# frgfm/Holocron

Measured on NVIDIA H100. Metric: images/sec RepVGG-A0 224^2 bf16 train, higher is better.
Workload: dtype bf16

## Files before the change

holocron_b200/csrc/conv_common.cuh:

```cuda
#pragma once
#include <cuda_runtime.h>
#include <type_traits>
#include "common.cuh"
#include "tc_common.cuh"
#include "tmap.cuh"

namespace conv {

constexpr int kThreads = 384;
constexpr int kConsumers = 256;

__device__ __forceinline__ void consumer_sync() { asm volatile("bar.sync 1, 256;" ::: "memory"); }

struct Ring {
  int stage = 0;
  uint32_t phase = 0;
  __device__ __forceinline__ void next(int n) {
    if (++stage == n) { stage = 0; phase ^= 1; }
  }
  __device__ __forceinline__ static Ring at(int k, int n) { return Ring{k % n, (uint32_t)(k / n) & 1}; }
};

__device__ __forceinline__ void add_residual16(uint4& val, const uint4& rv, bool relu) {
  __nv_bfloat162* a = reinterpret_cast<__nv_bfloat162*>(&val);
  const __nv_bfloat162* b = reinterpret_cast<const __nv_bfloat162*>(&rv);
#pragma unroll
  for (int jj = 0; jj < 4; ++jj) {
    float2 fa = __bfloat1622float2(a[jj]), fb = __bfloat1622float2(b[jj]);
    fa.x += fb.x; fa.y += fb.y;
    if (relu) { fa.x = hb::relu_nan(fa.x); fa.y = hb::relu_nan(fa.y); }
    a[jj] = __floats2bfloat162_rn(fa.x, fa.y);
  }
}

__device__ __forceinline__ void accum_pair(float4& s, const uint8_t* staged) {
  const float2 f = __bfloat1622float2(*reinterpret_cast<const __nv_bfloat162*>(staged));
  s.x += f.x; s.y += f.y; s.z = fmaf(f.x, f.x, s.z); s.w = fmaf(f.y, f.y, s.w);
}
__device__ __forceinline__ float2 fold_stats(const float4* scratch, int rgs, int npairs, int c) {
  const int pr = c >> 1, hi = c & 1;
  float sv = 0.f, qv = 0.f;
  for (int rg = 0; rg < rgs; ++rg) {
    const float4 v = scratch[rg * npairs + pr];
    sv += hi ? v.y : v.x;
    qv += hi ? v.w : v.z;
  }
  return make_float2(sv, qv);
}
__device__ __forceinline__ void store_stats(float* stats, int slot, int Cout, int channel, float2 v) {
  *reinterpret_cast<float2*>(stats + ((size_t)slot * Cout + channel) * 2) = v;
}

template <auto kKernel, typename... Args>
cudaError_t launch(int grid, size_t smem_bytes, cudaStream_t stream, const Args&... args) {
  static const cudaError_t attr =
      cudaFuncSetAttribute(kKernel, cudaFuncAttributeMaxDynamicSharedMemorySize, 227 * 1024);
  if (attr != cudaSuccess) return attr;
  kKernel<<<grid, kThreads, smem_bytes, stream>>>(args...);
  g_hb_launches.fetch_add(1, std::memory_order_relaxed);
  return cudaGetLastError();
}

template <int kStep, int kMax, int W = kStep, typename F>
cudaError_t dispatch_width(int w, F&& f) {
  if (w == W) return f(std::integral_constant<int, W>{});
  if constexpr (W + kStep <= kMax) return dispatch_width<kStep, kMax, W + kStep>(w, f);
  else return cudaErrorInvalidValue;
}

}

int hb_conv_rows_try(const void* x, const void* w, void* y, const float* bias, const void* residual, int N, int H, int W,
                     int Cin, int Cout, int act, int num_ctas, cudaStream_t stream, int nextra, const void* const* xe,
                     const void* const* we, float* stats, int* stat_slots);
int hb_wgrad_rows_try(const void* x, const void* dy, const void* dy1, float* ws, size_t ws_bytes, int N, int H, int W,
                      int Cin, int Cout, int num_ctas, cudaStream_t stream, int* slices_out);
size_t hb_wgrad_rows_workspace_bytes(int N, int H, int W, int Cin, int Cout, int R, int S, int stride, int pad, int dil,
                                     int num_ctas, int has_b1);
```

holocron_b200/csrc/conv_fprop.cu:

```cuda
#include <stdlib.h>
#include "conv_common.cuh"
#include "holocron_b200.h"

namespace {

using namespace tc;
using namespace conv;

constexpr int kBM = 128;
constexpr int kBK = 64;
constexpr int kMmaK = 16;
constexpr int kProducerRegs = 40;
constexpr int kConsumerRegs = 232;
constexpr int kABytes = kBM * kBK * 2;
constexpr int kSmemMax = 227 * 1024;

struct FpropParams {
  int m_total;
  int Ho, Wo;
  int stride, pad_h, pad_w, dil;
  int R, S;
  int Cin, Cout;
  int num_m_tiles, num_n_tiles;
  int cblocks;
  int ksteps_last;
  int e_mode, e_cblocks, e_ksteps_last;
  int nout;
  int stages;
  int b_stage_bytes;
  int out_pitch;
  int a_mode;
  int act;
  __nv_bfloat16* y;
  __nv_bfloat16* y2;
  float* stats;
  float* stats2;
  const float* bias;
  const __nv_bfloat16* residual;
  const float* norm_mean;
  const float* norm_rstd;
  const float* norm_wsum;
  int scatter, OH, OW, o_step, o_a, o_b;
};

template <bool kStats, int BN>
__global__ void __launch_bounds__(kThreads, 1)
conv_fprop_kernel(const __grid_constant__ CUtensorMap tmA, const __grid_constant__ CUtensorMap tmB,
                  const __grid_constant__ CUtensorMap tmA2, const __grid_constant__ CUtensorMap tmB2, const FpropParams p) {
  extern __shared__ __align__(1024) uint8_t smem_raw[];
  uint8_t* smem = reinterpret_cast<uint8_t*>((reinterpret_cast<uintptr_t>(smem_raw) + 1023) & ~uintptr_t(1023));
  const int stage_bytes = kABytes + p.b_stage_bytes;
  uint8_t* sout = smem + (size_t)p.stages * stage_bytes;
  const size_t sout_bytes = (((size_t)kBM * p.out_pitch + 15) & ~(size_t)15) + kBM * sizeof(long long);
  uint64_t* full_bar = reinterpret_cast<uint64_t*>(sout + sout_bytes);
  uint64_t* empty_bar = full_bar + p.stages;

  const int warp = threadIdx.x >> 5;
  const int lane = threadIdx.x & 31;

  if (warp == 0 && lane == 0) {
    prefetch_tmap(&tmA);
    prefetch_tmap(&tmB);
    if (p.e_mode) { prefetch_tmap(&tmB2); if (p.e_mode == 1) prefetch_tmap(&tmA2); }
    for (int i = 0; i < p.stages; ++i) { mbar_init(&full_bar[i], 1); mbar_init(&empty_bar[i], kConsumers / 32); }
    fence_barrier_init();
  }
  __syncthreads();

  const int n_tile = blockIdx.x % p.num_n_tiles;
  const int m_first = blockIdx.x / p.num_n_tiles, m_step = gridDim.x / p.num_n_tiles;
  const int kblocks = p.R * p.S * p.cblocks;
  const uint32_t tx_bytes = kABytes + BN * 128;

  if (warp < 4) {
    regs_release<kProducerRegs>();
    if (warp == 0 && lane == 0) {
      Ring ring;
      for (int m_tile = m_first; m_tile < p.num_m_tiles; m_tile += m_step) {
        const int m0 = m_tile * kBM;
        const int q0 = m0 % p.Wo, p0 = (m0 / p.Wo) % p.Ho, n0 = m0 / (p.Wo * p.Ho);
        const int base_w = q0 * p.stride - p.pad_w, base_h = p0 * p.stride - p.pad_h;
        for (int tap = 0; tap < p.R * p.S; ++tap) {
          const int r = tap / p.S, s = tap % p.S;
          for (int cb = 0; cb < p.cblocks; ++cb) {
            uint64_t* bar = &full_bar[ring.stage];
            mbar_wait(&empty_bar[ring.stage], ring.phase ^ 1);
            uint8_t* sa = smem + (size_t)ring.stage * stage_bytes;
            uint8_t* sb = sa + kABytes;
            mbar_arrive_expect_tx(bar, tx_bytes);
            if (p.a_mode == 1)
              tma_load_im2col_4d(&tmA, bar, sa, cb * kBK, base_w, base_h, n0, (uint16_t)(s * p.dil), (uint16_t)(r * p.dil));
            else
              tma_load_2d(&tmA, bar, sa, cb * kBK, m0);
            tma_load_3d(&tmB, bar, sb, cb * kBK, tap, n_tile * BN);
            ring.next(p.stages);
          }
        }
        for (int cb = 0; cb < p.e_cblocks; ++cb) {
          uint64_t* bar = &full_bar[ring.stage];
          mbar_wait(&empty_bar[ring.stage], ring.phase ^ 1);
          uint8_t* sa = smem + (size_t)ring.stage * stage_bytes;
          uint8_t* sb = sa + kABytes;
          mbar_arrive_expect_tx(bar, tx_bytes);
          if (p.e_mode == 1)
            tma_load_2d(&tmA2, bar, sa, cb * kBK, m0);
          else if (p.a_mode == 1)
            tma_load_im2col_4d(&tmA, bar, sa, cb * kBK, base_w, base_h, n0, (uint16_t)((p.S / 2) * p.dil),
                               (uint16_t)((p.R / 2) * p.dil));
          else
            tma_load_2d(&tmA, bar, sa, cb * kBK, m0);
          tma_load_3d(&tmB2, bar, sb, cb * kBK, 0, n_tile * BN);
          ring.next(p.stages);
        }
      }
    }
    return;
  }

  regs_acquire<kConsumerRegs>();
  const int et = threadIdx.x - 128;
  const int wg = et >> 7;
  const int wet = et & 127;
  const int frow = 64 * wg + frag_row(wet);
  const int fcol = frag_col(wet);
  const uint32_t dhi = desc_hi(1024);
  const uint32_t a_lo0 = desc_lo(smem_u32(smem), 16) + (uint32_t)wg * ((64 * 128) >> 4);
  const uint32_t stage_lo = (uint32_t)stage_bytes >> 4;
  long long* row_off = reinterpret_cast<long long*>(sout + (((size_t)kBM * p.out_pitch + 15) & ~(size_t)15));
  const int gpo = (BN + 63) >> 6;
  const int ngroups = p.nout * gpo;
  float4 st[4];
#pragma unroll
  for (int gi = 0; gi < 4; ++gi) st[gi] = make_float4(0.f, 0.f, 0.f, 0.f);
  const int col_base = n_tile * BN;
  const int ncols_valid = min(BN, p.Cout - col_base);
  constexpr int kCols = BN <= 64 ? 2 * BN : BN;
  float acc[kCols / 2];
  Ring ring;

  for (int m_tile = m_first; m_tile < p.num_m_tiles; m_tile += m_step) {
    int prev = -1;
    auto next_block = [&](uint32_t& a_lo, uint32_t& b_lo) {
      mbar_wait(&full_bar[ring.stage], ring.phase);
      a_lo = a_lo0 + (uint32_t)ring.stage * stage_lo;
      b_lo = desc_lo(smem_u32(smem), 16) + (uint32_t)ring.stage * stage_lo + (kABytes >> 4);
    };
    auto retire_prev = [&]() {
      wgmma_wait<1>();
      if (prev >= 0 && lane == 0) mbar_arrive(&empty_bar[prev]);
      prev = ring.stage;
      ring.next(p.stages);
    };
    for (int kb = 0, cb = 0; kb < kblocks; ++kb) {
      uint32_t a_lo, b_lo;
      next_block(a_lo, b_lo);
      if (++cb == p.cblocks) {
        cb = 0;
        wgmma_group_ks<BN, 0, 0>(p.ksteps_last, acc, a_lo, b_lo, 2, dhi, kb != 0);
      } else {
        wgmma_group<BN, kBK / kMmaK, 0, 0>(acc, a_lo, b_lo, 2, dhi, kb != 0);
      }
      retire_prev();
    }
    for (int ecb = 0; ecb < p.e_cblocks; ++ecb) {
      uint32_t a_lo, b_lo;
      next_block(a_lo, b_lo);
      const int ks = (ecb == p.e_cblocks - 1) ? p.e_ksteps_last : kBK / kMmaK;
      if constexpr (BN <= 64) {
        if (p.e_mode == 2) wgmma_group_ks<BN, 0, 0>(ks, acc + BN / 2, a_lo, b_lo, 2, dhi, ecb != 0);
        else wgmma_group_ks<BN, 0, 0>(ks, acc, a_lo, b_lo, 2, dhi, 1u);
      } else {
        wgmma_group_ks<BN, 0, 0>(ks, acc, a_lo, b_lo, 2, dhi, 1u);
      }
      retire_prev();
    }
    wgmma_wait<0>();
    fence_regs(acc);
    if (lane == 0) mbar_arrive(&empty_bar[prev]);

    const int rows_valid = min(kBM, p.m_total - m_tile * kBM);
    float nm[2] = {0.f, 0.f}, nr[2] = {1.f, 1.f};
    if (p.norm_mean) {
#pragma unroll
      for (int h = 0; h < 2; ++h) {
        const int m_row = m_tile * kBM + frow + 8 * h;
        if (m_row < p.m_total) { nm[h] = __ldg(p.norm_mean + m_row); nr[h] = __ldg(p.norm_rstd + m_row); }
      }
    }
#pragma unroll 1
    for (int gi = 0; gi < ngroups; ++gi) {
      const int o = gi >= gpo ? 1 : 0;
      const int g0 = (gi - o * gpo) * 64;
      const int gw = min(64, BN - g0);
      __nv_bfloat16* yo = o ? p.y2 : p.y;
      const bool first = o == 0;
      const int cs0 = o * BN + g0;
      consumer_sync();
      if (gi == 0 && et < kBM) {
        const long long m = (long long)m_tile * kBM + et;
        if (!p.scatter) {
          row_off[et] = m * p.Cout;
        } else {
          const int j = (int)(m % p.Wo), i = (int)((m / p.Wo) % p.Ho), n = (int)(m / ((long long)p.Wo * p.Ho));
          row_off[et] = (((long long)n * p.OH + (long long)i * p.o_step + p.o_a) * p.OW + (long long)j * p.o_step + p.o_b) * p.Cout;
        }
      }
#pragma unroll
      for (int j = 0; j < kCols / 8; ++j) {
        const int cs = 8 * j + fcol;
        if (cs >= cs0 && cs < cs0 + gw) {
          const int cl = cs - cs0;
          const int col = col_base + g0 + cl;
          const bool ok = col < p.Cout;
#pragma unroll
          for (int h = 0; h < 2; ++h) {
            float f0 = acc[4 * j + 2 * h], f1 = acc[4 * j + 2 * h + 1];
            if (first && p.norm_mean && ok) {
              f0 = nr[h] * (f0 - nm[h] * __ldg(p.norm_wsum + col));
              f1 = nr[h] * (f1 - nm[h] * __ldg(p.norm_wsum + col + 1));
            }
            if (first && p.bias && ok) { f0 += __ldg(p.bias + col); f1 += __ldg(p.bias + col + 1); }
            if (first && p.act == 1 && !p.residual) { f0 = hb::relu_nan(f0); f1 = hb::relu_nan(f1); }
            *reinterpret_cast<__nv_bfloat162*>(sout + (size_t)(frow + 8 * h) * p.out_pitch + cl * 2) =
                __floats2bfloat162_rn(f0, f1);
          }
        }
      }
      consumer_sync();
      const int chunks_per_row = gw / 8;
      const int total_chunks = rows_valid * chunks_per_row;
      int r = et / chunks_per_row, c8 = et - r * chunks_per_row;
      const int dr = kConsumers / chunks_per_row, dc = kConsumers - dr * chunks_per_row;
      const __nv_bfloat16* resid = first ? p.residual : nullptr;
      if (!resid) {
        for (int ch = et; ch < total_chunks; ch += kConsumers) {
          if (g0 + c8 * 8 < ncols_valid) {
            const uint4 val = *reinterpret_cast<const uint4*>(sout + (size_t)r * p.out_pitch + c8 * 16);
            *reinterpret_cast<uint4*>(yo + (size_t)row_off[r] + col_base + g0 + c8 * 8) = val;
          }
          r += dr; c8 += dc;
          if (c8 >= chunks_per_row) { c8 -= chunks_per_row; ++r; }
        }
      } else {
        for (int ch = et; ch < total_chunks; ch += 4 * kConsumers) {
          size_t off[4];
          int sidx[4];
          uint4 rv[4];
          bool ok[4];
#pragma unroll
          for (int u = 0; u < 4; ++u) {
            ok[u] = (ch + u * kConsumers < total_chunks) && (g0 + c8 * 8 < ncols_valid);
            sidx[u] = r * p.out_pitch + c8 * 16;
            off[u] = ok[u] ? (size_t)row_off[r] + col_base + g0 + c8 * 8 : 0;
            if (ok[u]) rv[u] = *reinterpret_cast<const uint4*>(resid + off[u]);
            r += dr; c8 += dc;
            if (c8 >= chunks_per_row) { c8 -= chunks_per_row; ++r; }
          }
#pragma unroll
          for (int u = 0; u < 4; ++u) {
            if (!ok[u]) continue;
            uint4 val = *reinterpret_cast<const uint4*>(sout + sidx[u]);
            add_residual16(val, rv[u], p.act == 1);
            *reinterpret_cast<uint4*>(yo + off[u]) = val;
          }
        }
      }
      if (kStats && (o ? (p.stats2 != nullptr) : (p.stats != nullptr))) {
        const int npairs = gw >> 1, rgs = 128 / npairs;
        const int rg = wet / npairs, pr = wet - rg * npairs;
        const int row_end = min(64 * wg + 64, rows_valid);
        if (rg < rgs && g0 + pr * 2 < ncols_valid) {
          const uint8_t* sp = sout + pr * 4;
          float4 s = make_float4(0.f, 0.f, 0.f, 0.f);
          for (int rr = 64 * wg + rg; rr < row_end; rr += rgs) accum_pair(s, sp + (size_t)rr * p.out_pitch);
#pragma unroll
          for (int g = 0; g < 4; ++g)
            if (g == gi) { st[g].x += s.x; st[g].y += s.y; st[g].z += s.z; st[g].w += s.w; }
        }
      }
    }
  }
  if (kStats && (p.stats || p.stats2)) {
    const int slot = (blockIdx.x / p.num_n_tiles) * 2 + wg;
#pragma unroll
    for (int gi = 0; gi < 4; ++gi) {
      if (gi >= ngroups) break;
      const int o = gi >= gpo ? 1 : 0;
      float* so = o ? p.stats2 : p.stats;
      if (!so) continue;
      const int g0 = (gi - o * gpo) * 64;
      const int gw = min(64, BN - g0);
      const int npairs = gw >> 1, rgs = 128 / npairs;
      consumer_sync();
      float4* scratch = reinterpret_cast<float4*>(sout) + wg * 128;
      scratch[wet] = st[gi];
      consumer_sync();
      if (wet < gw && g0 + wet < ncols_valid)
        store_stats(so, slot, p.Cout, col_base + g0 + wet, fold_stats(scratch, rgs, npairs, wet));
    }
  }
}

struct FpropArgs {
  const void* x; const void* w; void* y; const float* bias; const void* residual;
  int N, H, W, Cin, Cout, R, S, stride;
  int pad_h, pad_w, pad_after_h, pad_after_w, dil, act, num_ctas;
  int Ho, Wo;
  int scatter, OH, OW, o_step, o_a, o_b;
  const void* xe; const void* we; int Ce;
  const void* w2; void* y2;
  float* stats; float* stats2; int* stat_slots;
  const float* norm_mean; const float* norm_rstd; const float* norm_wsum;
  cudaStream_t stream;
};

int fprop_launch(const FpropArgs& a) {
  const int Cin = a.Cin, Cout = a.Cout, R = a.R, S = a.S;
  const long long m_total_ll = (long long)a.N * a.Ho * a.Wo;
  if (a.Ho <= 0 || a.Wo <= 0 || m_total_ll <= 0 || m_total_ll > 0x7fffffffLL) return (int)cudaErrorInvalidValue;
  const bool dual = a.w2 != nullptr;
  const bool kext = a.xe != nullptr;
  if (dual && kext) return (int)cudaErrorInvalidValue;
  if (dual && (!a.y2 || a.scatter || !(R & 1) || !(S & 1))) return (int)cudaErrorInvalidValue;
  if (kext && (!a.we || a.Ce % 8 != 0 || a.scatter || !hb::aligned16(a.xe) || !hb::aligned16(a.we)))
    return (int)cudaErrorInvalidValue;
  FpropParams p{};
  p.m_total = (int)m_total_ll;
  p.Ho = a.Ho; p.Wo = a.Wo;
  p.stride = a.stride; p.pad_h = a.pad_h; p.pad_w = a.pad_w; p.dil = a.dil;
  p.R = R; p.S = S; p.Cin = Cin; p.Cout = Cout;
  p.scatter = a.scatter; p.OH = a.OH; p.OW = a.OW; p.o_step = a.o_step; p.o_a = a.o_a; p.o_b = a.o_b;
  p.num_m_tiles = (p.m_total + kBM - 1) / kBM;
  int grid = a.num_ctas > 0 ? a.num_ctas : HB_NUM_SMS;
  if (grid > HB_NUM_SMS * 4) grid = HB_NUM_SMS * 4;
  const int bn_max = dual ? 64 : 128;
  int BN = Cout;
  if (Cout > bn_max) {
    BN = bn_max;
    for (int c = bn_max; c >= 64; c -= 16) if (Cout % c == 0) { BN = c; break; }
    const int wide = dual || R * S == 1 || a.stats ? 0 : Cout <= 256 ? Cout : Cout % 256 == 0 ? 256 : Cout % 192 == 0 ? 192 : 0;
    if (wide && (long long)p.num_m_tiles * (Cout / wide) >= grid) BN = wide;
  }
  p.nout = dual ? 2 : 1;
  p.num_n_tiles = (Cout + BN - 1) / BN;
  p.cblocks = (Cin + kBK - 1) / kBK;
  p.ksteps_last = ((Cin - (p.cblocks - 1) * kBK) + kMmaK - 1) / kMmaK;
  p.e_mode = kext ? 1 : (dual ? 2 : 0);
  const int ce = kext ? a.Ce : (dual ? Cin : 0);
  p.e_cblocks = (ce + kBK - 1) / kBK;
  p.e_ksteps_last = p.e_cblocks ? ((ce - (p.e_cblocks - 1) * kBK) + kMmaK - 1) / kMmaK : 0;
  p.b_stage_bytes = ((BN * 128) + 1023) & ~1023;
  p.out_pitch = (BN < 64 ? BN : 64) * 2 + 16;
  const int out_bytes = ((((kBM * p.out_pitch + 15) & ~15) + kBM * 8) + 1023) & ~1023;
  const int stage_bytes = kABytes + p.b_stage_bytes;
  int stages = (kSmemMax - 1024 - out_bytes - 2 * 8 * (int)sizeof(uint64_t)) / stage_bytes;
  if (stages > 8) stages = 8;
  if (stages < 2) return (int)cudaErrorInvalidValue;
  p.stages = stages;
  p.a_mode = (R == 1 && S == 1 && a.stride == 1 && a.pad_h == 0 && a.pad_w == 0 && a.pad_after_h == 0 &&
              a.pad_after_w == 0) ? 0 : 1;
  p.act = a.act;
  p.y = (__nv_bfloat16*)a.y;
  p.y2 = (__nv_bfloat16*)a.y2;
  p.stats = a.stats; p.stats2 = dual ? a.stats2 : nullptr;
  p.bias = a.bias;
  p.residual = (const __nv_bfloat16*)a.residual;
  p.norm_mean = a.norm_mean; p.norm_rstd = a.norm_rstd; p.norm_wsum = a.norm_wsum;
  if (p.norm_mean && (!p.norm_rstd || !p.norm_wsum || a.scatter)) return (int)cudaErrorInvalidValue;

  CUtensorMap tmA, tmB, tmA2, tmB2;
  int rc = p.a_mode == 0 ? tmap::encode_matrix(&tmA, a.x, p.m_total, Cin, kBM)
                         : tmap::encode_im2col_bf16(&tmA, a.x, a.N, a.H, a.W, Cin, a.pad_h, a.pad_w, R, S, a.dil,
                                                    a.stride, kBK, kBM, CU_TENSOR_MAP_SWIZZLE_128B, a.pad_after_h,
                                                    a.pad_after_w);
  if (rc) return rc;
  if ((rc = tmap::encode_krsc_slab(&tmB, a.w, Cout, R * S, Cin, BN))) return rc;
  tmA2 = tmA; tmB2 = tmB;
  if (kext && (rc = tmap::encode_matrix(&tmA2, a.xe, p.m_total, a.Ce, kBM))) return rc;
  if (p.e_mode && (rc = tmap::encode_krsc_slab(&tmB2, kext ? a.we : a.w2, Cout, 1, ce, BN))) return rc;

  const size_t smem_bytes = (size_t)stages * stage_bytes + out_bytes + 2 * stages * sizeof(uint64_t) + 1024;
  int per_n = grid / p.num_n_tiles;
  if (per_n < 1) per_n = 1;
  if (per_n > p.num_m_tiles) per_n = p.num_m_tiles;
  grid = per_n * p.num_n_tiles;
  if (a.stat_slots) *a.stat_slots = 2 * per_n;
  const bool stats = p.stats || p.stats2;
  return (int)dispatch_width<16, 256>(BN, [&](auto bn) {
    constexpr int kBN = decltype(bn)::value;
    if constexpr (kBN > 128) {
      if (stats) return cudaErrorInvalidValue;
      return launch<conv_fprop_kernel<false, kBN>>(grid, smem_bytes, a.stream, tmA, tmB, tmA2, tmB2, p);
    } else {
      return stats ? launch<conv_fprop_kernel<true, kBN>>(grid, smem_bytes, a.stream, tmA, tmB, tmA2, tmB2, p)
                   : launch<conv_fprop_kernel<false, kBN>>(grid, smem_bytes, a.stream, tmA, tmB, tmA2, tmB2, p);
    }
  });
}

}

extern "C" {

int hb_conv2d_fprop_bf16(const void* x, const void* w, void* y, const float* bias, const void* residual, int N, int H,
                         int W, int Cin, int Cout, int R, int S, int stride, int pad, int dil, int act, int num_ctas,
                         void* stream) {
  hb_conv_args a{};
  a.x = x; a.w = w; a.y = y; a.bias = bias; a.residual = residual;
  a.N = N; a.H = H; a.W = W; a.Cin = Cin; a.Cout = Cout; a.R = R; a.S = S; a.stride = stride; a.pad = pad; a.dil = dil;
  a.act = act; a.num_ctas = num_ctas;
  return hb_conv2d_fused_bf16(&a, nullptr, stream);
}

int hb_conv_stat_slots_max(void) { return 2 * HB_NUM_SMS * 4; }

int hb_conv2d_fused_bf16(const hb_conv_args* c, int* stat_slots, void* stream) {
  if (!c) return (int)cudaErrorInvalidValue;
  const int N = c->N, H = c->H, W = c->W, Cin = c->Cin, Cout = c->Cout, R = c->R, S = c->S;
  const int stride = c->stride, pad = c->pad, dil = c->dil;
  if (Cin % 8 != 0 || Cout % 16 != 0) return (int)cudaErrorInvalidValue;
  if (!hb::aligned16(c->x) || !hb::aligned16(c->w) || !hb::aligned16(c->y)) return (int)cudaErrorMisalignedAddress;
  if (c->w2 && (!hb::aligned16(c->w2) || !hb::aligned16(c->y2))) return (int)cudaErrorMisalignedAddress;
  const int Ho = (H + 2 * pad - dil * (R - 1) - 1) / stride + 1;
  const int Wo = (W + 2 * pad - dil * (S - 1) - 1) / stride + 1;
  if (Ho <= 0 || Wo <= 0) return (int)cudaErrorInvalidValue;
  if ((long long)N * Ho * Wo > 0x7fffffffLL) return (int)cudaErrorInvalidValue;
  if (c->w2 && pad != (R / 2) * dil) return (int)cudaErrorInvalidValue;
  if ((c->stats || c->stats2) && !stat_slots) return (int)cudaErrorInvalidValue;

  if (R == 3 && S == 3 && stride == 1 && pad == 1 && dil == 1 && !c->xe && !c->w2 && !c->norm_mean) {
    static const bool rows_enabled = getenv("HB_DISABLE_CONV_ROWS") == nullptr;
    if (rows_enabled) {
      const int rc = hb_conv_rows_try(c->x, c->w, c->y, c->bias, c->residual, N, H, W, Cin, Cout, c->act, c->num_ctas,
                                      (cudaStream_t)stream, 0, nullptr, nullptr, c->stats, stat_slots);
      if (rc != (int)cudaErrorNotSupported) return rc;
    }
  }
  FpropArgs a{};
  a.x = c->x; a.w = c->w; a.y = c->y; a.bias = c->bias; a.residual = c->residual;
  a.N = N; a.H = H; a.W = W; a.Cin = Cin; a.Cout = Cout; a.R = R; a.S = S; a.stride = stride;
  a.pad_h = a.pad_w = a.pad_after_h = a.pad_after_w = pad; a.dil = dil; a.act = c->act; a.num_ctas = c->num_ctas;
  a.Ho = Ho; a.Wo = Wo; a.stream = (cudaStream_t)stream;
  a.xe = c->xe; a.we = c->we; a.Ce = c->Ce; a.w2 = c->w2; a.y2 = c->y2;
  a.stats = c->stats; a.stats2 = c->stats2; a.stat_slots = stat_slots;
  a.norm_mean = c->norm_mean; a.norm_rstd = c->norm_rstd; a.norm_wsum = c->norm_wsum;
  return fprop_launch(a);
}

int hb_conv2d_dgrad_s2_bf16(const void* dy, const void* wcls, const void* dy1, const void* wd1, void* dx, int N, int H, int W,
                            int Ho, int Wo, int C, int Cd, int num_ctas, void* stream) {
  if (C % 8 != 0 || Cd % 16 != 0) return (int)cudaErrorInvalidValue;
  if (!hb::aligned16(dy) || !hb::aligned16(wcls) || !hb::aligned16(dx)) return (int)cudaErrorMisalignedAddress;
  if (Ho != (H - 1) / 2 + 1 || Wo != (W - 1) / 2 + 1 || H < 2 || W < 2) return (int)cudaErrorInvalidValue;
  const __nv_bfloat16* wc = (const __nv_bfloat16*)wcls;
  size_t woff = 0;
  for (int a = 0; a < 2; ++a) {
    for (int b = 0; b < 2; ++b) {
      const int Hc = (H - a + 1) / 2, Wc = (W - b + 1) / 2;
      const int R = 1 + a, S = 1 + b;
      FpropArgs f{};
      f.x = dy; f.w = wc + woff; f.y = dx; f.bias = nullptr; f.residual = nullptr;
      f.N = N; f.H = Ho; f.W = Wo; f.Cin = C; f.Cout = Cd; f.R = R; f.S = S; f.stride = 1;
      f.pad_h = 0; f.pad_w = 0;
      f.pad_after_h = a ? Hc + 1 - Ho : 0;
      f.pad_after_w = b ? Wc + 1 - Wo : 0;
      f.dil = 1; f.act = 0; f.num_ctas = num_ctas;
      f.Ho = Hc; f.Wo = Wc;
      f.scatter = 1; f.OH = H; f.OW = W; f.o_step = 2; f.o_a = a; f.o_b = b;
      f.stream = (cudaStream_t)stream;
      if (a == 0 && b == 0 && dy1 && wd1) {
        FpropArgs g = f;
        g.x = dy1; g.w = wd1;
        if (int rc = fprop_launch(g)) return rc;
        f.residual = dx;
      }
      if (Hc > 0 && Wc > 0) {
        if (int rc = fprop_launch(f)) return rc;
      }
      woff += (size_t)Cd * R * S * C;
    }
  }
  return 0;
}

}
```

holocron_b200/csrc/tc_common.cuh:

```cuda
#pragma once
#include <cuda.h>
#include <cuda_runtime.h>
#include <stdint.h>
#include "wgmma.cuh"

namespace tc {

__device__ __forceinline__ uint32_t smem_u32(const void* p) { return (uint32_t)__cvta_generic_to_shared(p); }

__device__ __forceinline__ bool elect_one() {
  uint32_t pred = 0;
  asm volatile(
      "{\n\t.reg .pred P;\n\t.reg .b32 R;\n\t"
      "elect.sync R|P, 0xffffffff;\n\t"
      "selp.b32 %0, 1, 0, P;\n\t}"
      : "=r"(pred));
  return pred != 0;
}

__device__ __forceinline__ void mbar_init(uint64_t* bar, uint32_t count) {
  asm volatile("mbarrier.init.shared::cta.b64 [%0], %1;" ::"r"(smem_u32(bar)), "r"(count));
}
__device__ __forceinline__ void fence_barrier_init() {
  asm volatile("fence.mbarrier_init.release.cluster;" ::: "memory");
}
__device__ __forceinline__ void fence_proxy_async() { asm volatile("fence.proxy.async.shared::cta;" ::: "memory"); }

__device__ __forceinline__ void mbar_arrive_expect_tx(uint64_t* bar, uint32_t bytes) {
  asm volatile("mbarrier.arrive.expect_tx.shared::cta.b64 _, [%0], %1;" ::"r"(smem_u32(bar)), "r"(bytes) : "memory");
}
__device__ __forceinline__ void mbar_arrive(uint64_t* bar) {
  asm volatile("mbarrier.arrive.shared::cta.b64 _, [%0];" ::"r"(smem_u32(bar)) : "memory");
}
__device__ __forceinline__ bool mbar_try_wait(uint64_t* bar, uint32_t parity) {
  uint32_t ok;
  asm volatile(
      "{\n\t.reg .pred P;\n\t"
      "mbarrier.try_wait.parity.shared::cta.b64 P, [%1], %2;\n\t"
      "selp.b32 %0, 1, 0, P;\n\t}"
      : "=r"(ok)
      : "r"(smem_u32(bar)), "r"(parity)
      : "memory");
  return ok != 0;
}
__device__ __forceinline__ void mbar_wait(uint64_t* bar, uint32_t parity) {
  uint32_t spins = 0;
  while (!mbar_try_wait(bar, parity)) {
    if (++spins > (1u << 26)) { asm volatile("trap;"); }
  }
}

__device__ __forceinline__ void prefetch_tmap(const CUtensorMap* m) {
  asm volatile("prefetch.tensormap [%0];" ::"l"(reinterpret_cast<uint64_t>(m)) : "memory");
}
__device__ __forceinline__ void tma_load_2d(const CUtensorMap* m, uint64_t* bar, void* dst, int c0, int c1) {
  asm volatile(
      "cp.async.bulk.tensor.2d.shared::cluster.global.mbarrier::complete_tx::bytes [%0], [%1, {%3, %4}], [%2];"
      ::"r"(smem_u32(dst)), "l"(reinterpret_cast<uint64_t>(m)), "r"(smem_u32(bar)), "r"(c0), "r"(c1)
      : "memory");
}
__device__ __forceinline__ void tma_load_3d(const CUtensorMap* m, uint64_t* bar, void* dst, int c0, int c1, int c2) {
  asm volatile(
      "cp.async.bulk.tensor.3d.shared::cluster.global.mbarrier::complete_tx::bytes [%0], [%1, {%3, %4, %5}], [%2];"
      ::"r"(smem_u32(dst)), "l"(reinterpret_cast<uint64_t>(m)), "r"(smem_u32(bar)), "r"(c0), "r"(c1), "r"(c2)
      : "memory");
}
__device__ __forceinline__ void tma_load_4d(const CUtensorMap* m, uint64_t* bar, void* dst, int c0, int c1, int c2,
                                            int c3) {
  asm volatile(
      "cp.async.bulk.tensor.4d.shared::cluster.global.mbarrier::complete_tx::bytes [%0], [%1, {%3, %4, %5, %6}], [%2];"
      ::"r"(smem_u32(dst)), "l"(reinterpret_cast<uint64_t>(m)), "r"(smem_u32(bar)), "r"(c0), "r"(c1), "r"(c2), "r"(c3)
      : "memory");
}
__device__ __forceinline__ void tma_load_im2col_4d(const CUtensorMap* m, uint64_t* bar, void* dst, int c, int w, int h,
                                                   int n, uint16_t off_w, uint16_t off_h) {
  asm volatile(
      "cp.async.bulk.tensor.4d.shared::cluster.global.im2col.mbarrier::complete_tx::bytes"
      " [%0], [%1, {%3, %4, %5, %6}], [%2], {%7, %8};"
      ::"r"(smem_u32(dst)), "l"(reinterpret_cast<uint64_t>(m)), "r"(smem_u32(bar)), "r"(c), "r"(w), "r"(h), "r"(n),
      "h"(off_w), "h"(off_h)
      : "memory");
}

__device__ __forceinline__ void wgmma_fence() { asm volatile("wgmma.fence.sync.aligned;" ::: "memory"); }
__device__ __forceinline__ void wgmma_commit() { asm volatile("wgmma.commit_group.sync.aligned;" ::: "memory"); }
template <int N>
__device__ __forceinline__ void wgmma_wait() { asm volatile("wgmma.wait_group.sync.aligned %0;" ::"n"(N) : "memory"); }
template <int N>
__device__ __forceinline__ void fence_regs(float (&r)[N]) {
#pragma unroll
  for (int i = 0; i < N; ++i) asm volatile("" : "+f"(r[i])::"memory");
}

template <int N>
__device__ __forceinline__ void regs_release() { asm volatile("setmaxnreg.dec.sync.aligned.u32 %0;" ::"n"(N)); }
template <int N>
__device__ __forceinline__ void regs_acquire() { asm volatile("setmaxnreg.inc.sync.aligned.u32 %0;" ::"n"(N)); }

__device__ __forceinline__ uint32_t desc_hi(uint32_t sbo_bytes) { return ((sbo_bytes >> 4) & 0x3FFF) | (1u << 30); }
__device__ __forceinline__ uint32_t desc_lo(uint32_t saddr, uint32_t lbo_bytes) {
  return ((saddr >> 4) & 0x3FFF) | (((lbo_bytes >> 4) & 0x3FFF) << 16);
}
__device__ __forceinline__ uint64_t make_desc(uint32_t lo, uint32_t hi) { return ((uint64_t)hi << 32) | lo; }

__device__ __forceinline__ int frag_row(int t) { return ((t >> 5) & 3) * 16 + ((t & 31) >> 2); }
__device__ __forceinline__ int frag_col(int t) { return (t & 3) * 2; }

template <int N, int KS, int TA, int TB>
__device__ __forceinline__ void wgmma_group(float* d, uint32_t a_lo, uint32_t b_lo, uint32_t step, uint32_t dhi,
                                            uint32_t scale_first) {
  wgmma_fence();
#pragma unroll
  for (int k = 0; k < KS; ++k)
    wgmma<N, TA, TB>(d, make_desc(a_lo + k * step, dhi), make_desc(b_lo + k * step, dhi), k ? 1u : scale_first);
  wgmma_commit();
}
template <int N, int TA, int TB>
__device__ __forceinline__ void wgmma_group_ks(int ks, float* d, uint32_t a_lo, uint32_t b_lo, uint32_t step,
                                               uint32_t dhi, uint32_t scale_first) {
  switch (ks) {
    case 1: wgmma_group<N, 1, TA, TB>(d, a_lo, b_lo, step, dhi, scale_first); break;
    case 2: wgmma_group<N, 2, TA, TB>(d, a_lo, b_lo, step, dhi, scale_first); break;
    case 3: wgmma_group<N, 3, TA, TB>(d, a_lo, b_lo, step, dhi, scale_first); break;
    default: wgmma_group<N, 4, TA, TB>(d, a_lo, b_lo, step, dhi, scale_first); break;
  }
}

}
```

Measured before the change: 9265.

## Add ping-pong consumer warpgroups to fprop conv kernel for epilogue overlap

For non-stats kernels with BN<=128, each consumer warpgroup now owns a whole 128-row M tile and the two warpgroups alternate tiles. Named barriers order their mainloops so one group's epilogue runs while the other issues WGMMAs. Each group gets its own output staging buffer, and the smem ring is skipped per tile to keep the stages in sync. The cost is double the accumulator registers per warpgroup and a larger staging area, which may reduce pipeline stages.

```diff
diff --git a/holocron_b200/csrc/conv_common.cuh b/holocron_b200/csrc/conv_common.cuh
--- a/holocron_b200/csrc/conv_common.cuh
+++ b/holocron_b200/csrc/conv_common.cuh
@@ -11,6 +11,10 @@
 constexpr int kConsumers = 256;
 
 __device__ __forceinline__ void consumer_sync() { asm volatile("bar.sync 1, 256;" ::: "memory"); }
+template <int kCount>
+__device__ __forceinline__ void bar_sync(int id) { asm volatile("bar.sync %0, %1;" ::"r"(id), "n"(kCount) : "memory"); }
+template <int kCount>
+__device__ __forceinline__ void bar_arrive(int id) { asm volatile("bar.arrive %0, %1;" ::"r"(id), "n"(kCount) : "memory"); }
 
 struct Ring {
   int stage = 0;
@@ -19,6 +23,12 @@
     if (++stage == n) { stage = 0; phase ^= 1; }
   }
   __device__ __forceinline__ static Ring at(int k, int n) { return Ring{k % n, (uint32_t)(k / n) & 1}; }
+  __device__ __forceinline__ void skip(int k, int n) {
+    stage += k;
+    const int q = stage / n;
+    stage -= q * n;
+    phase ^= (uint32_t)q & 1;
+  }
 };
 
 __device__ __forceinline__ void add_residual16(uint4& val, const uint4& rv, bool relu) {
diff --git a/holocron_b200/csrc/conv_fprop.cu b/holocron_b200/csrc/conv_fprop.cu
--- a/holocron_b200/csrc/conv_fprop.cu
+++ b/holocron_b200/csrc/conv_fprop.cu
@@ -43,16 +43,24 @@
   int scatter, OH, OW, o_step, o_a, o_b;
 };
 
+constexpr int kPingPongMaxBN = 128;
+__host__ __device__ constexpr size_t staging_bytes(int out_pitch) {
+  return (((size_t)kBM * out_pitch + 15) & ~(size_t)15) + kBM * sizeof(long long);
+}
+
 template <bool kStats, int BN>
 __global__ void __launch_bounds__(kThreads, 1)
 conv_fprop_kernel(const __grid_constant__ CUtensorMap tmA, const __grid_constant__ CUtensorMap tmB,
                   const __grid_constant__ CUtensorMap tmA2, const __grid_constant__ CUtensorMap tmB2, const FpropParams p) {
+  constexpr bool kPP = BN <= kPingPongMaxBN && !kStats;
+  constexpr int kHalves = kPP ? 2 : 1;
+  constexpr int kGroup = kPP ? 128 : 256;
   extern __shared__ __align__(1024) uint8_t smem_raw[];
   uint8_t* smem = reinterpret_cast<uint8_t*>((reinterpret_cast<uintptr_t>(smem_raw) + 1023) & ~uintptr_t(1023));
   const int stage_bytes = kABytes + p.b_stage_bytes;
   uint8_t* sout = smem + (size_t)p.stages * stage_bytes;
-  const size_t sout_bytes = (((size_t)kBM * p.out_pitch + 15) & ~(size_t)15) + kBM * sizeof(long long);
-  uint64_t* full_bar = reinterpret_cast<uint64_t*>(sout + sout_bytes);
+  const size_t sout_bytes = staging_bytes(p.out_pitch);
+  uint64_t* full_bar = reinterpret_cast<uint64_t*>(sout + kHalves * sout_bytes);
   uint64_t* empty_bar = full_bar + p.stages;
 
   const int warp = threadIdx.x >> 5;
@@ -62,7 +70,7 @@
     prefetch_tmap(&tmA);
     prefetch_tmap(&tmB);
     if (p.e_mode) { prefetch_tmap(&tmB2); if (p.e_mode == 1) prefetch_tmap(&tmA2); }
-    for (int i = 0; i < p.stages; ++i) { mbar_init(&full_bar[i], 1); mbar_init(&empty_bar[i], kConsumers / 32); }
+    for (int i = 0; i < p.stages; ++i) { mbar_init(&full_bar[i], 1); mbar_init(&empty_bar[i], kGroup / 32); }
     fence_barrier_init();
   }
   __syncthreads();
@@ -121,12 +129,17 @@
   const int et = threadIdx.x - 128;
   const int wg = et >> 7;
   const int wet = et & 127;
-  const int frow = 64 * wg + frag_row(wet);
+  const int gt = kPP ? wet : et;
+  const int group_bar = kPP ? 2 + wg : 1;
+  const int row0 = kPP ? 0 : 64 * wg;
+  const int frow = row0 + frag_row(wet);
   const int fcol = frag_col(wet);
   const uint32_t dhi = desc_hi(1024);
-  const uint32_t a_lo0 = desc_lo(smem_u32(smem), 16) + (uint32_t)wg * ((64 * 128) >> 4);
+  constexpr uint32_t kAHalf = (64 * 128) >> 4;
+  const uint32_t a_lo0 = desc_lo(smem_u32(smem), 16) + (uint32_t)row0 * (128 >> 4);
   const uint32_t stage_lo = (uint32_t)stage_bytes >> 4;
-  long long* row_off = reinterpret_cast<long long*>(sout + (((size_t)kBM * p.out_pitch + 15) & ~(size_t)15));
+  uint8_t* stg = sout + (kPP ? wg : 0) * sout_bytes;
+  long long* row_off = reinterpret_cast<long long*>(stg + (((size_t)kBM * p.out_pitch + 15) & ~(size_t)15));
   const int gpo = (BN + 63) >> 6;
   const int ngroups = p.nout * gpo;
   float4 st[4];
@@ -135,10 +148,15 @@
   const int col_base = n_tile * BN;
   const int ncols_valid = min(BN, p.Cout - col_base);
   constexpr int kCols = BN <= 64 ? 2 * BN : BN;
-  float acc[kCols / 2];
+  constexpr int kAccH = kCols / 2;
+  float acc[kHalves * kAccH];
   Ring ring;
-
-  for (int m_tile = m_first; m_tile < p.num_m_tiles; m_tile += m_step) {
+  const int stages_per_tile = kblocks + p.e_cblocks;
+  const int tile_step = kPP ? 2 * m_step : m_step;
+  if (kPP && wg == 1) ring.skip(stages_per_tile, p.stages);
+
+  for (int m_tile = m_first + (kPP ? wg * m_step : 0); m_tile < p.num_m_tiles; m_tile += tile_step) {
+    if (kPP && m_tile != m_first) bar_sync<256>(4 + wg);
     int prev = -1;
     auto next_block = [&](uint32_t& a_lo, uint32_t& b_lo) {
       mbar_wait(&full_bar[ring.stage], ring.phase);
@@ -156,9 +174,9 @@
       next_block(a_lo, b_lo);
       if (++cb == p.cblocks) {
         cb = 0;
-        wgmma_group_ks<BN, 0, 0>(p.ksteps_last, acc, a_lo, b_lo, 2, dhi, kb != 0);
+        wgmma_group_ks<BN, 0, 0, kHalves, kAccH>(p.ksteps_last, acc, a_lo, b_lo, 2, dhi, kb != 0, kAHalf);
       } else {
-        wgmma_group<BN, kBK / kMmaK, 0, 0>(acc, a_lo, b_lo, 2, dhi, kb != 0);
+        wgmma_group<BN, kBK / kMmaK, 0, 0, kHalves, kAccH>(acc, a_lo, b_lo, 2, dhi, kb != 0, kAHalf);
       }
       retire_prev();
     }
@@ -167,26 +185,20 @@
       next_block(a_lo, b_lo);
       const int ks = (ecb == p.e_cblocks - 1) ? p.e_ksteps_last : kBK / kMmaK;
       if constexpr (BN <= 64) {
-        if (p.e_mode == 2) wgmma_group_ks<BN, 0, 0>(ks, acc + BN / 2, a_lo, b_lo, 2, dhi, ecb != 0);
-        else wgmma_group_ks<BN, 0, 0>(ks, acc, a_lo, b_lo, 2, dhi, 1u);
+        if (p.e_mode == 2) wgmma_group_ks<BN, 0, 0, kHalves, kAccH>(ks, acc + BN / 2, a_lo, b_lo, 2, dhi, ecb != 0, kAHalf);
+        else wgmma_group_ks<BN, 0, 0, kHalves, kAccH>(ks, acc, a_lo, b_lo, 2, dhi, 1u, kAHalf);
       } else {
-        wgmma_group_ks<BN, 0, 0>(ks, acc, a_lo, b_lo, 2, dhi, 1u);
+        wgmma_group_ks<BN, 0, 0, kHalves, kAccH>(ks, acc, a_lo, b_lo, 2, dhi, 1u, kAHalf);
       }
       retire_prev();
     }
+    if (kPP && m_tile + m_step < p.num_m_tiles) bar_arrive<256>(5 - wg);
     wgmma_wait<0>();
     fence_regs(acc);
     if (lane == 0) mbar_arrive(&empty_bar[prev]);
+    if (kPP) ring.skip(stages_per_tile, p.stages);
 
     const int rows_valid = min(kBM, p.m_total - m_tile * kBM);
-    float nm[2] = {0.f, 0.f}, nr[2] = {1.f, 1.f};
-    if (p.norm_mean) {
-#pragma unroll
-      for (int h = 0; h < 2; ++h) {
-        const int m_row = m_tile * kBM + frow + 8 * h;
-        if (m_row < p.m_total) { nm[h] = __ldg(p.norm_mean + m_row); nr[h] = __ldg(p.norm_rstd + m_row); }
-      }
-    }
 #pragma unroll 1
     for (int gi = 0; gi < ngroups; ++gi) {
       const int o = gi >= gpo ? 1 : 0;
@@ -195,61 +207,72 @@
       __nv_bfloat16* yo = o ? p.y2 : p.y;
       const bool first = o == 0;
       const int cs0 = o * BN + g0;
-      consumer_sync();
-      if (gi == 0 && et < kBM) {
-        const long long m = (long long)m_tile * kBM + et;
+      bar_sync<kGroup>(group_bar);
+      if (gi == 0 && gt < kBM) {
+        const long long m = (long long)m_tile * kBM + gt;
         if (!p.scatter) {
-          row_off[et] = m * p.Cout;
+          row_off[gt] = m * p.Cout;
         } else {
           const int j = (int)(m % p.Wo), i = (int)((m / p.Wo) % p.Ho), n = (int)(m / ((long long)p.Wo * p.Ho));
-          row_off[et] = (((long long)n * p.OH + (long long)i * p.o_step + p.o_a) * p.OW + (long long)j * p.o_step + p.o_b) * p.Cout;
-        }
-      }
-#pragma unroll
-      for (int j = 0; j < kCols / 8; ++j) {
-        const int cs = 8 * j + fcol;
-        if (cs >= cs0 && cs < cs0 + gw) {
-          const int cl = cs - cs0;
-          const int col = col_base + g0 + cl;
-          const bool ok = col < p.Cout;
+          row_off[gt] = (((long long)n * p.OH + (long long)i * p.o_step + p.o_a) * p.OW + (long long)j * p.o_step + p.o_b) * p.Cout;
+        }
+      }
+#pragma unroll
+      for (int hh = 0; hh < kHalves; ++hh) {
+        float nm[2] = {0.f, 0.f}, nr[2] = {1.f, 1.f};
+        if (first && p.norm_mean) {
 #pragma unroll
           for (int h = 0; h < 2; ++h) {
-            float f0 = acc[4 * j + 2 * h], f1 = acc[4 * j + 2 * h + 1];
-            if (first && p.norm_mean && ok) {
-              f0 = nr[h] * (f0 - nm[h] * __ldg(p.norm_wsum + col));
-              f1 = nr[h] * (f1 - nm[h] * __ldg(p.norm_wsum + col + 1));
+            const int m_row = m_tile * kBM + frow + 64 * hh + 8 * h;
+            if (m_row < p.m_total) { nm[h] = __ldg(p.norm_mean + m_row); nr[h] = __ldg(p.norm_rstd + m_row); }
+          }
+        }
+#pragma unroll
+        for (int j = 0; j < kCols / 8; ++j) {
+          const int cs = 8 * j + fcol;
+          if (cs >= cs0 && cs < cs0 + gw) {
+            const int cl = cs - cs0;
+            const int col = col_base + g0 + cl;
+            const bool ok = col < p.Cout;
+#pragma unroll
+            for (int h = 0; h < 2; ++h) {
+              float f0 = acc[hh * kAccH + 4 * j + 2 * h], f1 = acc[hh * kAccH + 4 * j + 2 * h + 1];
+              if (first && p.norm_mean && ok) {
+                f0 = nr[h] * (f0 - nm[h] * __ldg(p.norm_wsum + col));
+                f1 = nr[h] * (f1 - nm[h] * __ldg(p.norm_wsum + col + 1));
+              }
+              if (first && p.bias && ok) { f0 += __ldg(p.bias + col); f1 += __ldg(p.bias + col + 1); }
+              if (first && p.act == 1 && !p.residual) { f0 = hb::relu_nan(f0); f1 = hb::relu_nan(f1); }
+              *reinterpret_cast<__nv_bfloat162*>(stg + (size_t)(frow + 64 * hh + 8 * h) * p.out_pitch + cl * 2) =
+                  __floats2bfloat162_rn(f0, f1);
             }
-            if (first && p.bias && ok) { f0 += __ldg(p.bias + col); f1 += __ldg(p.bias + col + 1); }
-            if (first && p.act == 1 && !p.residual) { f0 = hb::relu_nan(f0); f1 = hb::relu_nan(f1); }
-            *reinterpret_cast<__nv_bfloat162*>(sout + (size_t)(frow + 8 * h) * p.out_pitch + cl * 2) =
-                __floats2bfloat162_rn(f0, f1);
           }
         }
       }
-      consumer_sync();
+      bar_sync<kGroup>(group_bar);
       const int chunks_per_row = gw / 8;
       const int total_chunks = rows_valid * chunks_per_row;
-      int r = et / chunks_per_row, c8 = et - r * chunks_per_row;
-      const int dr = kConsumers / chunks_per_row, dc = kConsumers - dr * chunks_per_row;
+      int r = gt / chunks_per_row, c8 = gt - r * chunks_per_row;
+      const int dr = kGroup / chunks_per_row, dc = kGroup - dr * chunks_per_row;
       const __nv_bfloat16* resid = first ? p.residual : nullptr;
       if (!resid) {
-        for (int ch = et; ch < total_chunks; ch += kConsumers) {
+        for (int ch = gt; ch < total_chunks; ch += kGroup) {
           if (g0 + c8 * 8 < ncols_valid) {
-            const uint4 val = *reinterpret_cast<const uint4*>(sout + (size_t)r * p.out_pitch + c8 * 16);
+            const uint4 val = *reinterpret_cast<const uint4*>(stg + (size_t)r * p.out_pitch + c8 * 16);
             *reinterpret_cast<uint4*>(yo + (size_t)row_off[r] + col_base + g0 + c8 * 8) = val;
           }
           r += dr; c8 += dc;
           if (c8 >= chunks_per_row) { c8 -= chunks_per_row; ++r; }
         }
       } else {
-        for (int ch = et; ch < total_chunks; ch += 4 * kConsumers) {
+        for (int ch = gt; ch < total_chunks; ch += 4 * kGroup) {
           size_t off[4];
           int sidx[4];
           uint4 rv[4];
           bool ok[4];
 #pragma unroll
           for (int u = 0; u < 4; ++u) {
-            ok[u] = (ch + u * kConsumers < total_chunks) && (g0 + c8 * 8 < ncols_valid);
+            ok[u] = (ch + u * kGroup < total_chunks) && (g0 + c8 * 8 < ncols_valid);
             sidx[u] = r * p.out_pitch + c8 * 16;
             off[u] = ok[u] ? (size_t)row_off[r] + col_base + g0 + c8 * 8 : 0;
             if (ok[u]) rv[u] = *reinterpret_cast<const uint4*>(resid + off[u]);
@@ -259,7 +282,7 @@
 #pragma unroll
           for (int u = 0; u < 4; ++u) {
             if (!ok[u]) continue;
-            uint4 val = *reinterpret_cast<const uint4*>(sout + sidx[u]);
+            uint4 val = *reinterpret_cast<const uint4*>(stg + sidx[u]);
             add_residual16(val, rv[u], p.act == 1);
             *reinterpret_cast<uint4*>(yo + off[u]) = val;
           }
@@ -270,7 +293,7 @@
         const int rg = wet / npairs, pr = wet - rg * npairs;
         const int row_end = min(64 * wg + 64, rows_valid);
         if (rg < rgs && g0 + pr * 2 < ncols_valid) {
-          const uint8_t* sp = sout + pr * 4;
+          const uint8_t* sp = stg + pr * 4;
           float4 s = make_float4(0.f, 0.f, 0.f, 0.f);
           for (int rr = 64 * wg + rg; rr < row_end; rr += rgs) accum_pair(s, sp + (size_t)rr * p.out_pitch);
 #pragma unroll
@@ -351,7 +374,8 @@
   p.e_ksteps_last = p.e_cblocks ? ((ce - (p.e_cblocks - 1) * kBK) + kMmaK - 1) / kMmaK : 0;
   p.b_stage_bytes = ((BN * 128) + 1023) & ~1023;
   p.out_pitch = (BN < 64 ? BN : 64) * 2 + 16;
-  const int out_bytes = ((((kBM * p.out_pitch + 15) & ~15) + kBM * 8) + 1023) & ~1023;
+  const bool stats = a.stats || (dual && a.stats2);
+  const int out_bytes = ((BN <= kPingPongMaxBN && !stats ? 2 : 1) * (int)staging_bytes(p.out_pitch) + 1023) & ~1023;
   const int stage_bytes = kABytes + p.b_stage_bytes;
   int stages = (kSmemMax - 1024 - out_bytes - 2 * 8 * (int)sizeof(uint64_t)) / stage_bytes;
   if (stages > 8) stages = 8;
@@ -385,7 +409,6 @@
   if (per_n > p.num_m_tiles) per_n = p.num_m_tiles;
   grid = per_n * p.num_n_tiles;
   if (a.stat_slots) *a.stat_slots = 2 * per_n;
-  const bool stats = p.stats || p.stats2;
   return (int)dispatch_width<16, 256>(BN, [&](auto bn) {
     constexpr int kBN = decltype(bn)::value;
     if constexpr (kBN > 128) {
diff --git a/holocron_b200/csrc/tc_common.cuh b/holocron_b200/csrc/tc_common.cuh
--- a/holocron_b200/csrc/tc_common.cuh
+++ b/holocron_b200/csrc/tc_common.cuh
@@ -106,23 +106,26 @@
 __device__ __forceinline__ int frag_row(int t) { return ((t >> 5) & 3) * 16 + ((t & 31) >> 2); }
 __device__ __forceinline__ int frag_col(int t) { return (t & 3) * 2; }
 
-template <int N, int KS, int TA, int TB>
+template <int N, int KS, int TA, int TB, int MH = 1, int DS = 0>
 __device__ __forceinline__ void wgmma_group(float* d, uint32_t a_lo, uint32_t b_lo, uint32_t step, uint32_t dhi,
-                                            uint32_t scale_first) {
+                                            uint32_t scale_first, uint32_t a_half = 0) {
   wgmma_fence();
 #pragma unroll
   for (int k = 0; k < KS; ++k)
-    wgmma<N, TA, TB>(d, make_desc(a_lo + k * step, dhi), make_desc(b_lo + k * step, dhi), k ? 1u : scale_first);
+#pragma unroll
+    for (int h = 0; h < MH; ++h)
+      wgmma<N, TA, TB>(d + h * DS, make_desc(a_lo + h * a_half + k * step, dhi), make_desc(b_lo + k * step, dhi),
+                       k ? 1u : scale_first);
   wgmma_commit();
 }
-template <int N, int TA, int TB>
+template <int N, int TA, int TB, int MH = 1, int DS = 0>
 __device__ __forceinline__ void wgmma_group_ks(int ks, float* d, uint32_t a_lo, uint32_t b_lo, uint32_t step,
-                                               uint32_t dhi, uint32_t scale_first) {
+                                               uint32_t dhi, uint32_t scale_first, uint32_t a_half = 0) {
   switch (ks) {
-    case 1: wgmma_group<N, 1, TA, TB>(d, a_lo, b_lo, step, dhi, scale_first); break;
-    case 2: wgmma_group<N, 2, TA, TB>(d, a_lo, b_lo, step, dhi, scale_first); break;
-    case 3: wgmma_group<N, 3, TA, TB>(d, a_lo, b_lo, step, dhi, scale_first); break;
-    default: wgmma_group<N, 4, TA, TB>(d, a_lo, b_lo, step, dhi, scale_first); break;
+    case 1: wgmma_group<N, 1, TA, TB, MH, DS>(d, a_lo, b_lo, step, dhi, scale_first, a_half); break;
+    case 2: wgmma_group<N, 2, TA, TB, MH, DS>(d, a_lo, b_lo, step, dhi, scale_first, a_half); break;
+    case 3: wgmma_group<N, 3, TA, TB, MH, DS>(d, a_lo, b_lo, step, dhi, scale_first, a_half); break;
+    default: wgmma_group<N, 4, TA, TB, MH, DS>(d, a_lo, b_lo, step, dhi, scale_first, a_half); break;
   }
 }
 
```

New measurement: 9327 (median of 6 runs). No clear change (+0.7%).
